# uzh-rpg/rpg_svo

Measured on AMD Instinct MI355X. Metric: frames/sec sparse-align+pose-refine (VGA, 4 pyr lvls); ATE vs CPU ref, higher is better.
Workload: dtype value = default build: K1 f32 pixels/residuals/chi2/per-pixel products, f64 Jacobian rows/partials/reductions/projection/solve/pose; K4 f64 (reference-width build: roofline_f64_build.value)

## Files before the change

rpg_svo_amd/csrc/pose_optimizer_wave.hip:

```cpp
#include "track_kernels.h"
#include "track_math.h"
#include "wave_reduce.h"

using namespace svo_capi;
using namespace svo_dev;

namespace {

using svo_track::PoseWaveArgs;

constexpr int PW_WAVES = 4;
constexpr int PW_MINW = 3;
constexpr double SVO_EPS = 0.0000000001;


__device__ __forceinline__ double uni(double v) {
  const uint32_t l = (uint32_t)__builtin_amdgcn_readfirstlane((int)lo32(v));
  const uint32_t h = (uint32_t)__builtin_amdgcn_readfirstlane((int)hi32(v));
  return mk_f64(l, h);
}
__device__ __forceinline__ void uni_se3(Se3& T) {
#pragma unroll
  for (int k = 0; k < 4; ++k) T.q[k] = uni(T.q[k]);
#pragma unroll
  for (int k = 0; k < 3; ++k) T.t[k] = uni(T.t[k]);
}


__device__ __forceinline__ double wave_reduce32_f64(const double v[32], int lane) {
  double r[16], q[8], t[4], u[2];
#pragma unroll
  for (int k = 0; k < 16; ++k) r[k] = swap32_add(v[k], v[k + 16]);
#pragma unroll
  for (int k = 0; k < 8; ++k) q[k] = swap16_add(r[k], r[k + 8]);
  {
    const bool hi = (lane & 8) != 0;
#pragma unroll
    for (int k = 0; k < 4; ++k) {
      const double mine = hi ? q[k + 4] : q[k], send = hi ? q[k] : q[k + 4];
      t[k] = mine + dpp_f64<DPP_ROW_ROR8>(send);
    }
  }
  {
    const bool hi = (lane & 4) != 0;
#pragma unroll
    for (int k = 0; k < 2; ++k) {
      const double mine = hi ? t[k + 2] : t[k], send = hi ? t[k] : t[k + 2];
      u[k] = mine + dpp_f64<DPP_ROW_HALF_MIRROR>(send);
    }
  }
  const bool hi = (lane & 2) != 0;
  const double mine = hi ? u[1] : u[0], send = hi ? u[0] : u[1];
  double w = mine + dpp_f64<DPP_QUAD_XOR2>(send);
  w += dpp_f64<DPP_QUAD_XOR1>(w);
  return w;
}

__device__ __forceinline__ double fast_rcp(double z) {
  double r = __builtin_amdgcn_rcp(z);
  r = fma(fma(-z, r, 1.0), r, r);
  r = fma(fma(-z, r, 1.0), r, r);
  return r;
}
__device__ __forceinline__ double fast_sqrt(double x) {
  const double r = __builtin_amdgcn_rsq(x);
  double g = x * r;
  const double h = 0.5 * r;
  g = fma(fma(-g, g, x), h, g);
  g = fma(fma(-g, g, x), h, g);
  return fmax(g, 0.0);
}

__device__ __forceinline__ void ldlt6_factor_fast(const double H[21], double LD[21]) {
  double d[6];
#pragma unroll
  for (int j = 0; j < 6; ++j) {
    double dj = H[sym6(j, j)];
#pragma unroll
    for (int k = 0; k < j; ++k) dj -= LD[low6(j, k)] * LD[low6(j, k)] * d[k];
    d[j] = dj;
    const bool ok = fabs(dj) > 2.2250738585072014e-308;
    const double inv = ok ? fast_rcp(dj) : 0.0;
    LD[15 + j] = inv;
#pragma unroll
    for (int i = j + 1; i < 6; ++i) {
      double v = H[sym6(j, i)];
#pragma unroll
      for (int k = 0; k < j; ++k) v -= LD[low6(i, k)] * LD[low6(j, k)] * d[k];
      LD[low6(i, j)] = v * inv;
    }
  }
}

__device__ __forceinline__ void se3_exp_fast(const double xi[6], double q[4], double t[3]) {
  const double ox = xi[3], oy = xi[4], oz = xi[5];
  const double theta_sq = ox * ox + oy * oy + oz * oz;
  const double theta = fast_sqrt(theta_sq);
  double s_h, c_h;
  sincos_small(0.5 * theta, &s_h, &c_h);
  const double ux = xi[0], uy = xi[1], uz = xi[2];
  if (theta < 1e-10) {
    const double theta_po4 = theta_sq * theta_sq;
    const double imag_factor = 0.5 - 0.0208333 * theta_sq + 0.000260417 * theta_po4;
    q[0] = c_h; q[1] = imag_factor * ox; q[2] = imag_factor * oy; q[3] = imag_factor * oz;
    quat_rot(q, xi, t);
  } else {
    const double it = fast_rcp(theta);
    const double imag_factor = s_h * it;
    q[0] = c_h; q[1] = imag_factor * ox; q[2] = imag_factor * oy; q[3] = imag_factor * oz;
    const double it2 = it * it;
    const double s_t = 2.0 * s_h * c_h;
    const double c1 = (2.0 * s_h * s_h) * it2;
    const double c2 = (theta - s_t) * (it2 * it);
    const double wx = oy * uz - oz * uy, wy = oz * ux - ox * uz, wz = ox * uy - oy * ux;
    const double wwx = oy * wz - oz * wy, wwy = oz * wx - ox * wz, wwz = ox * wy - oy * wx;
    t[0] = ux + c1 * wx + c2 * wwx;
    t[1] = uy + c1 * wy + c2 * wwy;
    t[2] = uz + c1 * wz + c2 * wwz;
  }
}

__device__ __forceinline__ Se3 se3_compose_fast(const Se3& a, const Se3& b) {
  Se3 r;
  double rt[3];
  quat_rot(a.q, b.t, rt);
  r.t[0] = a.t[0] + rt[0]; r.t[1] = a.t[1] + rt[1]; r.t[2] = a.t[2] + rt[2];
  quat_mul(a.q, b.q, r.q);
  quat_normalize_fast(r.q);
  return r;
}

__device__ __forceinline__ float tukey_w(float x) {
  const float b_square = 4.6851f * 4.6851f;
  const float x_square = x * x;
  const float tmp = 1.0f - x_square / b_square;
  return (x_square <= b_square) ? tmp * tmp : 0.0f;
}

template <int NPL, typename K>
__device__ __forceinline__ K radix_select(const K key[NPL], int k, int top_bit) {
  K prefix = 0;
  int cnt_lo = 0, cnt_hi = NPL * 64;
  for (int bit = top_bit; bit >= 0; --bit) {
    const K cand = prefix | ((K)1 << bit);
    int cnt = 0;
#pragma unroll
    for (int j = 0; j < NPL; ++j) cnt += __popcll(__ballot(key[j] < cand));
    if (cnt <= k) {
      prefix = cand;
      cnt_lo = cnt;
    } else {
      cnt_hi = cnt;
    }
    if (cnt_hi - cnt_lo == 1 && bit > 0) {
      const K upper = prefix + ((K)1 << bit);
      K found = prefix;
#pragma unroll
      for (int j = 0; j < NPL; ++j) {
        const unsigned long long m = __ballot(key[j] >= prefix && key[j] < upper);
        if (m) {
          const int src = __ffsll((long long)m) - 1;
          if (sizeof(K) == 8) {
            const unsigned lo = __builtin_amdgcn_readlane((int)(unsigned)key[j], src);
            const unsigned hi = __builtin_amdgcn_readlane((int)(unsigned)((unsigned long long)key[j] >> 32), src);
            found = (K)(((unsigned long long)hi << 32) | lo);
          } else {
            found = (K)(unsigned)__builtin_amdgcn_readlane((int)(unsigned)key[j], src);
          }
        }
      }
      return found;
    }
  }
  return prefix;
}

__device__ __forceinline__ bool pivots_ok(const double A[21], const double LD[21]) {
  double dmax = 0.0, imax = 0.0;
  bool zero = false;
#pragma unroll
  for (int k = 0; k < 6; ++k) {
    dmax = fmax(dmax, fabs(A[sym6(k, k)]));
    const double id = fabs(LD[15 + k]);
    zero = zero || !(id > 0.0);
    imax = fmax(imax, id);
  }
  return !zero && (imax * dmax * 1e-9 < 1.0);
}

template <int J>
__device__ __forceinline__ double bcast(double v) { return readlane_f64<2 * J>(v); }

template <int NPL>
__global__ void __launch_bounds__(64 * PW_WAVES, PW_MINW) pose_opt_wave_kernel(const PoseWaveArgs a) {
  const int lane = threadIdx.x & 63;
  const int b = blockIdx.x * PW_WAVES + (threadIdx.x >> 6);
  if (b >= a.B) return;
  int n = a.n[b];
  n = n < 0 ? 0 : (n > a.n_stride ? a.n_stride : n);
  const size_t base = (size_t)b * a.n_stride;
  const double focal = fabs(a.cam.fx);

  double px[NPL], py[NPL], pz[NPL], ux[NPL], uy[NPL];
  float kk[NPL];
  bool live[NPL];
  int n_err = 0;
#pragma unroll
  for (int j = 0; j < NPL; ++j) {
    const int i = j * 64 + lane;
    live[j] = (i < n) && a.has_point[base + i] != 0;
    px[j] = py[j] = 0.0;
    pz[j] = 1.0;
    ux[j] = uy[j] = 0.0;
    kk[j] = 1.f;
    if (live[j]) {
      const double* p = a.pos + 3 * (base + i);
      const double* f = a.f + 3 * (base + i);
      px[j] = p[0]; py[j] = p[1]; pz[j] = p[2];
      ux[j] = f[0] / f[2];
      uy[j] = f[1] / f[2];
      kk[j] = pow2_inv_f32(a.level[base + i]);
    }
    n_err += __popcll(__ballot(live[j]));
  }
  if (n_err == 0) {
    if (lane == 0) a.ran[b] = 0;
    return;
  }

  Se3 T, T_old;
  se3_from_Rt(a.T + 12 * b, T);
  uni_se3(T);
  T_old = T;
  double R[9];
  quat_to_R(T.q, R);
#pragma unroll
  for (int k = 0; k < 9; ++k) R[k] = uni(R[k]);

  double estimated_scale, med_init;
  {
    unsigned long long kd[NPL];
#pragma unroll
    for (int j = 0; j < NPL; ++j) {
      const double x = R[0] * px[j] + R[1] * py[j] + R[2] * pz[j] + T.t[0];
      const double y = R[3] * px[j] + R[4] * py[j] + R[5] * pz[j] + T.t[1];
      const double z = R[6] * px[j] + R[7] * py[j] + R[8] * pz[j] + T.t[2];
      const double k = (double)kk[j];
      const double zi = fast_rcp(z);
      const double e0 = (ux[j] - x * zi) * k, e1 = (uy[j] - y * zi) * k;
      const double e2 = e0 * e0 + e1 * e1;
      kd[j] = live[j] ? (unsigned long long)__double_as_longlong(e2) : 0x7ff0000000000000ull;
    }
    med_init = __longlong_as_double((long long)radix_select<NPL, unsigned long long>(kd, n_err / 2, 62));
    const float median_f = (float)sqrt(med_init);
    estimated_scale = (double)(1.48f * median_f);
  }

  double scale = estimated_scale;
  double chi2 = 0.0;
  if (a.n_iter == 0) {
    if (lane == 0) a.ran[b] = 2;
    return;
  }
  for (int iter = 0; iter < a.n_iter; ++iter) {
    if (iter == 5) scale = 0.85 / focal;
    const double inv_scale = 1.0 / scale;
    double A[21];
    double acc[32];
#pragma unroll
    for (int k = 0; k < 32; ++k) acc[k] = 0.0;
#pragma unroll
    for (int j = 0; j < NPL; ++j) {
      const double x = R[0] * px[j] + R[1] * py[j] + R[2] * pz[j] + T.t[0];
      const double y = R[3] * px[j] + R[4] * py[j] + R[5] * pz[j] + T.t[1];
      const double z = R[6] * px[j] + R[7] * py[j] + R[8] * pz[j] + T.t[2];
      const double zi = fast_rcp(z);
      const double xn = x * zi, yn = y * zi;
      const double k = (double)kk[j];
      const double e0 = (ux[j] - xn) * k, e1 = (uy[j] - yn) * k;
      const double e2 = e0 * e0 + e1 * e1;
      const float wf = tukey_w((float)(fast_sqrt(e2) * inv_scale));
      const double w = live[j] ? (double)wf : 0.0;
      const double j00 = -zi * k, j02 = xn * zi * k, j03 = xn * yn * k, j04 = -(1.0 + xn * xn) * k, j05 = yn * k;
      const double j11 = -zi * k, j12 = yn * zi * k, j13 = (1.0 + yn * yn) * k, j14 = -j03, j15 = -xn * k;
      const double w00 = w * j00, w02 = w * j02, w03 = w * j03, w04 = w * j04, w05 = w * j05;
      const double w11 = w * j11, w12 = w * j12, w13 = w * j13, w14 = w * j14, w15 = w * j15;
      acc[0] = fma(w00, j00, acc[0]);
      acc[1] = fma(w00, j02, acc[1]);
      acc[2] = fma(w00, j03, acc[2]);
      acc[3] = fma(w00, j04, acc[3]);
      acc[4] = fma(w00, j05, acc[4]);
      acc[5] = fma(w11, j11, acc[5]);
      acc[6] = fma(w11, j12, acc[6]);
      acc[7] = fma(w11, j13, acc[7]);
      acc[8] = fma(w11, j14, acc[8]);
      acc[9] = fma(w11, j15, acc[9]);
      acc[10] = fma(w02, j02, fma(w12, j12, acc[10]));
      acc[11] = fma(w02, j03, fma(w12, j13, acc[11]));
      acc[12] = fma(w02, j04, fma(w12, j14, acc[12]));
      acc[13] = fma(w02, j05, fma(w12, j15, acc[13]));
      acc[14] = fma(w03, j03, fma(w13, j13, acc[14]));
      acc[15] = fma(w03, j04, fma(w13, j14, acc[15]));
      acc[16] = fma(w03, j05, fma(w13, j15, acc[16]));
      acc[17] = fma(w04, j04, fma(w14, j14, acc[17]));
      acc[18] = fma(w04, j05, fma(w14, j15, acc[18]));
      acc[19] = fma(w05, j05, fma(w15, j15, acc[19]));
      acc[20] = fma(-w00, e0, acc[20]);
      acc[21] = fma(-w11, e1, acc[21]);
      acc[22] = fma(-w02, e0, fma(-w12, e1, acc[22]));
      acc[23] = fma(-w03, e0, fma(-w13, e1, acc[23]));
      acc[24] = fma(-w04, e0, fma(-w14, e1, acc[24]));
      acc[25] = fma(-w05, e0, fma(-w15, e1, acc[25]));
      acc[26] = fma(e2, w, acc[26]);
    }
    const double tot = wave_reduce32_f64(acc, lane);
    const double s0 = bcast<0>(tot), s1 = bcast<1>(tot), s2 = bcast<2>(tot), s3 = bcast<3>(tot), s4 = bcast<4>(tot);
    const double s5 = bcast<5>(tot), s6 = bcast<6>(tot), s7 = bcast<7>(tot), s8 = bcast<8>(tot), s9 = bcast<9>(tot);
    const double s10 = bcast<10>(tot), s11 = bcast<11>(tot), s12 = bcast<12>(tot), s13 = bcast<13>(tot);
    const double s14 = bcast<14>(tot), s15 = bcast<15>(tot), s16 = bcast<16>(tot), s17 = bcast<17>(tot);
    const double s18 = bcast<18>(tot), s19 = bcast<19>(tot);
    const double bv[6] = {bcast<20>(tot), bcast<21>(tot), bcast<22>(tot), bcast<23>(tot), bcast<24>(tot), bcast<25>(tot)};
    const double new_chi2 = bcast<26>(tot);
    A[sym6(0, 0)] = s0; A[sym6(0, 1)] = 0.0; A[sym6(0, 2)] = s1; A[sym6(0, 3)] = s2; A[sym6(0, 4)] = s3; A[sym6(0, 5)] = s4;
    A[sym6(1, 1)] = s5; A[sym6(1, 2)] = s6; A[sym6(1, 3)] = s7; A[sym6(1, 4)] = s8; A[sym6(1, 5)] = s9;
    A[sym6(2, 2)] = s10; A[sym6(2, 3)] = s11; A[sym6(2, 4)] = s12; A[sym6(2, 5)] = s13;
    A[sym6(3, 3)] = s14; A[sym6(3, 4)] = s15; A[sym6(3, 5)] = s16;
    A[sym6(4, 4)] = s17; A[sym6(4, 5)] = s18; A[sym6(5, 5)] = s19;

    double dT[6];
    double LD[21];
    ldlt6_factor_fast(A, LD);
    if (!pivots_ok(A, LD)) {
      if (lane == 0) a.ran[b] = 2;
      return;
    }
    ldlt6_solve(LD, bv, dT);

    bool last = false;
    if ((iter > 0 && new_chi2 > chi2) || isnan(dT[0])) {
      T = T_old;
      last = true;
    } else {
      Se3 ex;
      se3_exp_fast(dT, ex.q, ex.t);
      T_old = T;
      T = se3_compose_fast(ex, T);
      uni_se3(T);
      chi2 = new_chi2;
      double nm = 0.0;
#pragma unroll
      for (int k = 0; k < 6; ++k) nm = fmax(nm, fabs(dT[k]));
      last = nm <= SVO_EPS;
    }
    quat_to_R(T.q, R);
#pragma unroll
    for (int k = 0; k < 9; ++k) R[k] = uni(R[k]);
    last = last || iter + 1 == a.n_iter;
    if (last) {
      if (a.Cov) {
        double e[6], x[6];
#pragma unroll
        for (int i = 0; i < 6; ++i) e[i] = (i == lane) ? 1.0 : 0.0;
        ldlt6_solve(LD, e, x);
        const double if2 = 1.0 / (focal * focal);
        if (lane < 6) {
#pragma unroll
          for (int i = 0; i < 6; ++i) a.Cov[36 * b + i * 6 + lane] = x[i] * if2;
        }
      }
      break;
    }
  }
  if (lane == 0) se3_to_Rt(T, a.T + 12 * b);

  const double reproj_thresh_scaled = a.reproj_thresh / focal;
  const double reproj_thresh2 = reproj_thresh_scaled * reproj_thresh_scaled;
  int n_deleted = 0;
  double med_final;
  {
    unsigned long long kd[NPL];
#pragma unroll
    for (int j = 0; j < NPL; ++j) {
      const double x = R[0] * px[j] + R[1] * py[j] + R[2] * pz[j] + T.t[0];
      const double y = R[3] * px[j] + R[4] * py[j] + R[5] * pz[j] + T.t[1];
      const double z = R[6] * px[j] + R[7] * py[j] + R[8] * pz[j] + T.t[2];
      const double k = (double)kk[j];
      const double zi = fast_rcp(z);
      const double e0 = (ux[j] - x * zi) * k, e1 = (uy[j] - y * zi) * k;
      const double e2 = e0 * e0 + e1 * e1;
      kd[j] = live[j] ? (unsigned long long)__double_as_longlong(e2) : 0x7ff0000000000000ull;
      const bool prune = live[j] && e2 > reproj_thresh2;
      if (prune) a.has_point[base + j * 64 + lane] = 0;
      n_deleted += __popcll(__ballot(prune));
    }
    med_final = __longlong_as_double((long long)radix_select<NPL, unsigned long long>(kd, n_err / 2, 62));
  }
  if (lane == 0) {
    a.stats[4 * b + 0] = estimated_scale * focal;
    a.stats[4 * b + 1] = a.n_iter > 0 ? sqrt(med_init) * focal : 0.0;
    a.stats[4 * b + 2] = sqrt(med_final) * focal;
    a.stats[4 * b + 3] = (double)(n_err - n_deleted);
    a.ran[b] = 1;
  }
}

}

namespace svo_track {

int launch_pose_wave(const PoseWaveArgs& a, hipStream_t s) {
  const int grid = (a.B + PW_WAVES - 1) / PW_WAVES;
  const dim3 g(grid), blk(64 * PW_WAVES);
  if (a.n_stride <= 64) hipLaunchKernelGGL(pose_opt_wave_kernel<1>, g, blk, 0, s, a);
  else if (a.n_stride <= 128) hipLaunchKernelGGL(pose_opt_wave_kernel<2>, g, blk, 0, s, a);
  else hipLaunchKernelGGL(pose_opt_wave_kernel<4>, g, blk, 0, s, a);
  return check_launch();
}

}
```

Before: 11.52 million.

## Compact live observations into per-wave LDS and loop over live trips only

Per-observation data no longer sits in register arrays sized by a compile-time NPL. Each wave now stream-compacts its live observations into dynamic LDS in a structure-of-arrays layout, keeps slot indices so pruning can still write back, and loops only over the live trips. It also drops the redundant Jacobian accumulators (j11 equals j00 and j14 equals -j03, so three sums are reconstructed from others) and raises min waves per EU from 3 to 4. The aim is lower register pressure, higher occupancy and skipping dead lanes, at the cost of LDS traffic on every iteration and a runtime-trip loop that is no longer unrolled.

New measurement: 11.67 million (median of 6 runs). +1.3%, better.

```diff
diff --git a/rpg_svo_amd/csrc/pose_optimizer_wave.hip b/rpg_svo_amd/csrc/pose_optimizer_wave.hip
--- a/rpg_svo_amd/csrc/pose_optimizer_wave.hip
+++ b/rpg_svo_amd/csrc/pose_optimizer_wave.hip
@@ -10,7 +10,7 @@
 using svo_track::PoseWaveArgs;
 
 constexpr int PW_WAVES = 4;
-constexpr int PW_MINW = 3;
+constexpr int PW_MINW = 4;
 constexpr double SVO_EPS = 0.0000000001;
 
 
@@ -191,42 +191,84 @@
 template <int J>
 __device__ __forceinline__ double bcast(double v) { return readlane_f64<2 * J>(v); }
 
-template <int NPL>
+struct PwObs {
+  double px, py, pz, ux, uy, k;
+};
+
+struct PwBlock {
+  double* d;
+  float* k;
+  uint8_t* slot;
+  int cap;
+  __device__ __forceinline__ PwObs load(int c) const {
+    PwObs o;
+    o.px = d[c]; o.py = d[cap + c]; o.pz = d[2 * cap + c]; o.ux = d[3 * cap + c]; o.uy = d[4 * cap + c];
+    o.k = (double)k[c];
+    return o;
+  }
+};
+constexpr int PW_BYTES_PER_OBS = 5 * 8 + 4 + 1;
+__host__ __device__ constexpr int pw_cap(int n_stride) { return (n_stride + 7) & ~7; }
+
+__device__ __forceinline__ double pw_e2(const PwObs& o, const double R[9], const double t[3]) {
+  const double x = R[0] * o.px + R[1] * o.py + R[2] * o.pz + t[0];
+  const double y = R[3] * o.px + R[4] * o.py + R[5] * o.pz + t[1];
+  const double z = R[6] * o.px + R[7] * o.py + R[8] * o.pz + t[2];
+  const double zi = fast_rcp(z);
+  const double e0 = (o.ux - x * zi) * o.k, e1 = (o.uy - y * zi) * o.k;
+  return e0 * e0 + e1 * e1;
+}
+
+__device__ __forceinline__ double pw_select(const unsigned long long kd[4], int trips, int k) {
+  unsigned long long r;
+  if (trips <= 1) r = radix_select<1, unsigned long long>(kd, k, 62);
+  else if (trips == 2) r = radix_select<2, unsigned long long>(kd, k, 62);
+  else if (trips == 3) r = radix_select<3, unsigned long long>(kd, k, 62);
+  else r = radix_select<4, unsigned long long>(kd, k, 62);
+  return __longlong_as_double((long long)r);
+}
+
 __global__ void __launch_bounds__(64 * PW_WAVES, PW_MINW) pose_opt_wave_kernel(const PoseWaveArgs a) {
+  SVO_DYNAMIC_LDS(double, pw_dyn);
   const int lane = threadIdx.x & 63;
-  const int b = blockIdx.x * PW_WAVES + (threadIdx.x >> 6);
+  const int wave = threadIdx.x >> 6;
+  const int b = blockIdx.x * PW_WAVES + wave;
   if (b >= a.B) return;
-  int n = a.n[b];
+  int n = __builtin_amdgcn_readfirstlane(a.n[b]);
   n = n < 0 ? 0 : (n > a.n_stride ? a.n_stride : n);
   const size_t base = (size_t)b * a.n_stride;
   const double focal = fabs(a.cam.fx);
 
-  double px[NPL], py[NPL], pz[NPL], ux[NPL], uy[NPL];
-  float kk[NPL];
-  bool live[NPL];
-  int n_err = 0;
-#pragma unroll
-  for (int j = 0; j < NPL; ++j) {
+  PwBlock blk;
+  blk.cap = pw_cap(a.n_stride);
+  blk.d = pw_dyn + (size_t)wave * (blk.cap / 8) * PW_BYTES_PER_OBS;
+  blk.k = reinterpret_cast<float*>(blk.d + 5 * blk.cap);
+  blk.slot = reinterpret_cast<uint8_t*>(blk.k + blk.cap);
+  int n_live = 0;
+  for (int j = 0; j * 64 < n; ++j) {
     const int i = j * 64 + lane;
-    live[j] = (i < n) && a.has_point[base + i] != 0;
-    px[j] = py[j] = 0.0;
-    pz[j] = 1.0;
-    ux[j] = uy[j] = 0.0;
-    kk[j] = 1.f;
-    if (live[j]) {
+    const bool live = (i < n) && a.has_point[base + i] != 0;
+    const unsigned long long m = __ballot(live);
+    if (live) {
+      const int at = n_live + __popcll(m & ((1ull << lane) - 1ull));
+      const int c = at < blk.cap ? at : blk.cap - 1;
       const double* p = a.pos + 3 * (base + i);
       const double* f = a.f + 3 * (base + i);
-      px[j] = p[0]; py[j] = p[1]; pz[j] = p[2];
-      ux[j] = f[0] / f[2];
-      uy[j] = f[1] / f[2];
-      kk[j] = pow2_inv_f32(a.level[base + i]);
-    }
-    n_err += __popcll(__ballot(live[j]));
-  }
-  if (n_err == 0) {
+      blk.d[c] = p[0]; blk.d[blk.cap + c] = p[1]; blk.d[2 * blk.cap + c] = p[2];
+      blk.d[3 * blk.cap + c] = f[0] / f[2];
+      blk.d[4 * blk.cap + c] = f[1] / f[2];
+      blk.k[c] = pow2_inv_f32(a.level[base + i]);
+      blk.slot[c] = (uint8_t)i;
+    }
+    n_live += __popcll(m);
+  }
+  if (n_live == 0) {
     if (lane == 0) a.ran[b] = 0;
     return;
   }
+  SVO_WAVE_LDS_FENCE();
+  const int last_pos = (n_live < blk.cap ? n_live : blk.cap) - 1;
+  const int trips = (n_live + 63) >> 6;
 
   Se3 T, T_old;
   se3_from_Rt(a.T + 12 * b, T);
@@ -239,19 +281,17 @@
 
   double estimated_scale, med_init;
   {
-    unsigned long long kd[NPL];
-#pragma unroll
-    for (int j = 0; j < NPL; ++j) {
-      const double x = R[0] * px[j] + R[1] * py[j] + R[2] * pz[j] + T.t[0];
-      const double y = R[3] * px[j] + R[4] * py[j] + R[5] * pz[j] + T.t[1];
-      const double z = R[6] * px[j] + R[7] * py[j] + R[8] * pz[j] + T.t[2];
-      const double k = (double)kk[j];
-      const double zi = fast_rcp(z);
-      const double e0 = (ux[j] - x * zi) * k, e1 = (uy[j] - y * zi) * k;
-      const double e2 = e0 * e0 + e1 * e1;
-      kd[j] = live[j] ? (unsigned long long)__double_as_longlong(e2) : 0x7ff0000000000000ull;
-    }
-    med_init = __longlong_as_double((long long)radix_select<NPL, unsigned long long>(kd, n_err / 2, 62));
+    unsigned long long kd[4];
+#pragma unroll
+    for (int j = 0; j < 4; ++j) {
+      kd[j] = 0x7ff0000000000000ull;
+      if (j < trips) {
+        const int at = j * 64 + lane;
+        const double e2 = pw_e2(blk.load(at < last_pos ? at : last_pos), R, T.t);
+        if (at < n_live) kd[j] = (unsigned long long)__double_as_longlong(e2);
+      }
+    }
+    med_init = pw_select(kd, trips, n_live / 2);
     const float median_f = (float)sqrt(med_init);
     estimated_scale = (double)(1.48f * median_f);
   }
@@ -269,31 +309,31 @@
     double acc[32];
 #pragma unroll
     for (int k = 0; k < 32; ++k) acc[k] = 0.0;
-#pragma unroll
-    for (int j = 0; j < NPL; ++j) {
-      const double x = R[0] * px[j] + R[1] * py[j] + R[2] * pz[j] + T.t[0];
-      const double y = R[3] * px[j] + R[4] * py[j] + R[5] * pz[j] + T.t[1];
-      const double z = R[6] * px[j] + R[7] * py[j] + R[8] * pz[j] + T.t[2];
+#pragma unroll 1
+    for (int j = 0; j < trips; ++j) {
+      const int at = j * 64 + lane;
+      const PwObs o = blk.load(at < last_pos ? at : last_pos);
+      const double x = R[0] * o.px + R[1] * o.py + R[2] * o.pz + T.t[0];
+      const double y = R[3] * o.px + R[4] * o.py + R[5] * o.pz + T.t[1];
+      const double z = R[6] * o.px + R[7] * o.py + R[8] * o.pz + T.t[2];
       const double zi = fast_rcp(z);
       const double xn = x * zi, yn = y * zi;
-      const double k = (double)kk[j];
-      const double e0 = (ux[j] - xn) * k, e1 = (uy[j] - yn) * k;
+      const double k = o.k;
+      const double e0 = (o.ux - xn) * k, e1 = (o.uy - yn) * k;
       const double e2 = e0 * e0 + e1 * e1;
       const float wf = tukey_w((float)(fast_sqrt(e2) * inv_scale));
-      const double w = live[j] ? (double)wf : 0.0;
+      const double w = at < n_live ? (double)wf : 0.0;
       const double j00 = -zi * k, j02 = xn * zi * k, j03 = xn * yn * k, j04 = -(1.0 + xn * xn) * k, j05 = yn * k;
-      const double j11 = -zi * k, j12 = yn * zi * k, j13 = (1.0 + yn * yn) * k, j14 = -j03, j15 = -xn * k;
+      const double j12 = yn * zi * k, j13 = (1.0 + yn * yn) * k, j14 = -j03, j15 = -xn * k;
       const double w00 = w * j00, w02 = w * j02, w03 = w * j03, w04 = w * j04, w05 = w * j05;
-      const double w11 = w * j11, w12 = w * j12, w13 = w * j13, w14 = w * j14, w15 = w * j15;
+      const double w11 = w00, w12 = w * j12, w13 = w * j13, w14 = w * j14, w15 = w * j15;
       acc[0] = fma(w00, j00, acc[0]);
       acc[1] = fma(w00, j02, acc[1]);
       acc[2] = fma(w00, j03, acc[2]);
       acc[3] = fma(w00, j04, acc[3]);
       acc[4] = fma(w00, j05, acc[4]);
-      acc[5] = fma(w11, j11, acc[5]);
       acc[6] = fma(w11, j12, acc[6]);
       acc[7] = fma(w11, j13, acc[7]);
-      acc[8] = fma(w11, j14, acc[8]);
       acc[9] = fma(w11, j15, acc[9]);
       acc[10] = fma(w02, j02, fma(w12, j12, acc[10]));
       acc[11] = fma(w02, j03, fma(w12, j13, acc[11]));
@@ -315,14 +355,14 @@
     }
     const double tot = wave_reduce32_f64(acc, lane);
     const double s0 = bcast<0>(tot), s1 = bcast<1>(tot), s2 = bcast<2>(tot), s3 = bcast<3>(tot), s4 = bcast<4>(tot);
-    const double s5 = bcast<5>(tot), s6 = bcast<6>(tot), s7 = bcast<7>(tot), s8 = bcast<8>(tot), s9 = bcast<9>(tot);
+    const double s6 = bcast<6>(tot), s7 = bcast<7>(tot), s9 = bcast<9>(tot);
     const double s10 = bcast<10>(tot), s11 = bcast<11>(tot), s12 = bcast<12>(tot), s13 = bcast<13>(tot);
     const double s14 = bcast<14>(tot), s15 = bcast<15>(tot), s16 = bcast<16>(tot), s17 = bcast<17>(tot);
     const double s18 = bcast<18>(tot), s19 = bcast<19>(tot);
     const double bv[6] = {bcast<20>(tot), bcast<21>(tot), bcast<22>(tot), bcast<23>(tot), bcast<24>(tot), bcast<25>(tot)};
     const double new_chi2 = bcast<26>(tot);
     A[sym6(0, 0)] = s0; A[sym6(0, 1)] = 0.0; A[sym6(0, 2)] = s1; A[sym6(0, 3)] = s2; A[sym6(0, 4)] = s3; A[sym6(0, 5)] = s4;
-    A[sym6(1, 1)] = s5; A[sym6(1, 2)] = s6; A[sym6(1, 3)] = s7; A[sym6(1, 4)] = s8; A[sym6(1, 5)] = s9;
+    A[sym6(1, 1)] = s0; A[sym6(1, 2)] = s6; A[sym6(1, 3)] = s7; A[sym6(1, 4)] = -s2; A[sym6(1, 5)] = s9;
     A[sym6(2, 2)] = s10; A[sym6(2, 3)] = s11; A[sym6(2, 4)] = s12; A[sym6(2, 5)] = s13;
     A[sym6(3, 3)] = s14; A[sym6(3, 4)] = s15; A[sym6(3, 5)] = s16;
     A[sym6(4, 4)] = s17; A[sym6(4, 5)] = s18; A[sym6(5, 5)] = s19;
@@ -378,28 +418,31 @@
   int n_deleted = 0;
   double med_final;
   {
-    unsigned long long kd[NPL];
-#pragma unroll
-    for (int j = 0; j < NPL; ++j) {
-      const double x = R[0] * px[j] + R[1] * py[j] + R[2] * pz[j] + T.t[0];
-      const double y = R[3] * px[j] + R[4] * py[j] + R[5] * pz[j] + T.t[1];
-      const double z = R[6] * px[j] + R[7] * py[j] + R[8] * pz[j] + T.t[2];
-      const double k = (double)kk[j];
-      const double zi = fast_rcp(z);
-      const double e0 = (ux[j] - x * zi) * k, e1 = (uy[j] - y * zi) * k;
-      const double e2 = e0 * e0 + e1 * e1;
-      kd[j] = live[j] ? (unsigned long long)__double_as_longlong(e2) : 0x7ff0000000000000ull;
-      const bool prune = live[j] && e2 > reproj_thresh2;
-      if (prune) a.has_point[base + j * 64 + lane] = 0;
-      n_deleted += __popcll(__ballot(prune));
-    }
-    med_final = __longlong_as_double((long long)radix_select<NPL, unsigned long long>(kd, n_err / 2, 62));
+    unsigned long long kd[4];
+#pragma unroll
+    for (int j = 0; j < 4; ++j) {
+      kd[j] = 0x7ff0000000000000ull;
+      if (j < trips) {
+        const int at = j * 64 + lane;
+        const int c = at < last_pos ? at : last_pos;
+        const double e2 = pw_e2(blk.load(c), R, T.t);
+        const bool live = at < n_live;
+        if (live) kd[j] = (unsigned long long)__double_as_longlong(e2);
+        const bool prune = live && e2 > reproj_thresh2;
+        if (prune) {
+          const int slot = blk.slot[c];
+          if (slot < n) a.has_point[base + slot] = 0;
+        }
+        n_deleted += __popcll(__ballot(prune));
+      }
+    }
+    med_final = pw_select(kd, trips, n_live / 2);
   }
   if (lane == 0) {
     a.stats[4 * b + 0] = estimated_scale * focal;
     a.stats[4 * b + 1] = a.n_iter > 0 ? sqrt(med_init) * focal : 0.0;
     a.stats[4 * b + 2] = sqrt(med_final) * focal;
-    a.stats[4 * b + 3] = (double)(n_err - n_deleted);
+    a.stats[4 * b + 3] = (double)(n_live - n_deleted);
     a.ran[b] = 1;
   }
 }
@@ -410,10 +453,8 @@
 
 int launch_pose_wave(const PoseWaveArgs& a, hipStream_t s) {
   const int grid = (a.B + PW_WAVES - 1) / PW_WAVES;
-  const dim3 g(grid), blk(64 * PW_WAVES);
-  if (a.n_stride <= 64) hipLaunchKernelGGL(pose_opt_wave_kernel<1>, g, blk, 0, s, a);
-  else if (a.n_stride <= 128) hipLaunchKernelGGL(pose_opt_wave_kernel<2>, g, blk, 0, s, a);
-  else hipLaunchKernelGGL(pose_opt_wave_kernel<4>, g, blk, 0, s, a);
+  const size_t lds = (size_t)PW_WAVES * pw_cap(a.n_stride) * PW_BYTES_PER_OBS;
+  hipLaunchKernelGGL(pose_opt_wave_kernel, dim3(grid), dim3(64 * PW_WAVES), lds, s, a);
   return check_launch();
 }
 
```
